# tugitbartlomiej/ViTParticleFilterTracker

Measured on AMD Instinct MI355X. Metric: frames/sec @ 4096 particles, ViT-B/16 224px; 1/2/4/8 MI355X scaling, higher is better.
Workload: dtype bf16; 1 GPU; 4096 particles, vit_base_patch16_224 bf16, 224x224 frames, full tracking step per frame; particles=4096, particles_per_gpu=4096, arch=vit_base_patch16_224, hip_graph=True, parallelism=particle-shard x1

## Files before the change

### vitparticlefiltertracker_amd/csrc/gemm_bf16.hip

```cpp
#include <algorithm>
#include <atomic>
#include "gemm_common.h"

using namespace vpf;
using namespace vpf::gemm;

namespace {

constexpr int BK = 64;
constexpr int OPERAND_BYTES = BM * BK * 2;
static_assert(OPERAND_BYTES == TILE_BYTES, "bf16 K-tile geometry");
constexpr int AUX_PARTS = 15;
constexpr int MAX_PARTS = 16;
constexpr int AUX_BYTES = 2048 + AUX_PARTS * 2048;

template <int EPI, bool WIDE = false, bool OUT8 = false, bool PART = false>
__global__ __launch_bounds__(NTHREADS) void k_gemm_bf16(const bf16_t* __restrict__ A, int lda,
                                                        const bf16_t* __restrict__ W,
                                                        const float* __restrict__ bias,
                                                        const bf16_t* residual,
                                                        const float* __restrict__ pos, int g2,
                                                        const float2* __restrict__ stats,
                                                        const float* __restrict__ colsum,
                                                        bf16_t* C, int ldc, int M, int N, int K, int group,
// ... 120 lines not shown
        }
        return;
    }
    if constexpr (LN) {
        if constexpr (wide) {
            asm volatile("s_waitcnt vmcnt(0)" ::: "memory");
            __builtin_amdgcn_s_barrier();
            asm volatile("" ::: "memory");
        }
        combine_planes(planes_lds, aux, stats_parts, K, ln_eps, tid);
    }
    const int region = (wid >> 1) + ((wid >> 1) >= (nk % 3) ? 1 : 0);
    finish_tile<EPI, OUT8, DIRECT>(smem + region * OPERAND_BYTES + (wid & 1) * 16384, aux, acc, wm, wn, m0, n0, lane,
                                   residual, pos, g2, C, ldc, M, N, stats_out, stats_rows, o8);
}

template <int EPI, bool OUT8 = false>
__global__ __launch_bounds__(NTHREADS) void k_gemm_pp(const bf16_t* __restrict__ A, int lda,
                                                      const bf16_t* __restrict__ W,
                                                      const float* __restrict__ bias,
                                                      const bf16_t* residual,
                                                      const float* __restrict__ pos, int g2,
                                                      const float2* __restrict__ stats,
                                                      const float* __restrict__ colsum,
                                                      bf16_t* C, int ldc, int M, int N, int K, int group,
                                                      int stats_parts, float ln_eps, float* stats_out,
                                                      int stats_rows, Out8 o8) {
    constexpr int HALF = 16384;
    constexpr int RING = 8 * HALF;
    static_assert(RING + AUX_BYTES <= 160 * 1024, "LDS budget");
    __shared__ __attribute__((aligned(16))) char smem[RING + AUX_BYTES];
    const int tid = threadIdx.x, lane = tid & 63;
    const int wid = __builtin_amdgcn_readfirstlane(tid >> 6);
    const int wm = wid >> 2, wn = wid & 3;

    int m0, n0;
    tile_of(M, N, group, m0, n0);
    constexpr bool DIRECT = (EPI == VPF_EPI_LN_GELU || EPI == VPF_EPI_BIAS_GELU) && !OUT8;

    const char* Ablk = reinterpret_cast<const char*>(A) + (size_t)m0 * lda * 2;
    const char* Bblk = reinterpret_cast<const char*>(W) + (size_t)n0 * K * 2;
    uint32_t off[4][2];
#pragma unroll
    for (int p = 0; p < 2; ++p) {
        const int rho = (wid + 8 * p) * 8 + (lane >> 3);
        const int lch = (lane & 7) ^ ((rho >> 1) & 7);
        const int ra0 = (rho >> 6) * 128 + (rho & 63);
        const int rb0 = (rho >> 5) * 64 + (DIRECT ? wperm(rho & 31) : (rho & 31));
        const int ra[2] = {ra0, ra0 + 64}, rb[2] = {rb0, rb0 + 32};
#pragma unroll
        for (int h = 0; h < 2; ++h) {
            off[h == 0 ? 0 : 3][p] = (uint32_t)min(ra[h], M - 1 - m0) * (uint32_t)(lda * 2) + (uint32_t)(lch * 16);
            off[h == 0 ? 1 : 2][p] = (uint32_t)min(rb[h], N - 1 - n0) * (uint32_t)(K * 2) + (uint32_t)(lch * 16);
        }
    }
    const int nk = K / BK;
    auto stage = [&](int type, int kt) {
        kt = min(kt, nk - 1);
        char* slot = smem + ((kt & 1) * 4 + type) * HALF;
        const char* src = (type == 0 || type == 3) ? Ablk : Bblk;
        const uint32_t koff = (uint32_t)kt * (BK * 2);
#pragma unroll
        for (int p = 0; p < 2; ++p)
            __builtin_amdgcn_global_load_lds((gptr_t)(src + off[type][p] + koff), (lptr_t)(slot + (wid + 8 * p) * 1024),
                                             16, 0, 0);
    };

    constexpr bool LN = (EPI == VPF_EPI_LN || EPI == VPF_EPI_LN_GELU);
    char* aux = smem + RING;
    dma_bias_colsum<LN>(aux, bias, colsum, n0, N, wid, lane);
    if constexpr (LN) dma_planes(aux + 2048, stats, stats_parts, m0, M, wid, lane);
    stage(0, 0); stage(1, 0); stage(2, 0); stage(3, 0); stage(0, 1); stage(1, 1);
    asm volatile("s_waitcnt vmcnt(8)" ::: "memory");
    __builtin_amdgcn_s_barrier();
    if (wm == 1) __builtin_amdgcn_s_barrier();
    asm volatile("" ::: "memory");

    f32x4 acc[4][8];
#pragma unroll
    for (int j = 0; j < 4; ++j)
#pragma unroll
        for (int i = 0; i < 8; ++i) acc[j][i] = f32x4{0.f, 0.f, 0.f, 0.f};

    const int fr = lane & 15, fq = lane >> 4;
    const int sw = (fr >> 1) & 7;
    const int abase = (wm * 64 + fr) * 128, bbase = (wn * 32 + fr) * 128;
    auto mfma_quadrant = [&](const i32x4 (&fa)[2][4], const i32x4 (&fb)[2][2], int mh, int nh) {
        asm volatile("s_waitcnt lgkmcnt(0)" ::: "memory");
        __builtin_amdgcn_sched_barrier(0);
#pragma unroll
        for (int ks = 0; ks < 2; ++ks)
#pragma unroll
            for (int j = 0; j < 2; ++j)
#pragma unroll
                for (int i = 0; i < 4; ++i)
                    acc[nh * 2 + j][mh * 4 + i] = __builtin_amdgcn_mfma_f32_16x16x32_bf16(
                        __builtin_bit_cast(bf16x8, fb[ks][j]), __builtin_bit_cast(bf16x8, fa[ks][i]),
                        acc[nh * 2 + j][mh * 4 + i], 0, 0, 0);
        __builtin_amdgcn_sched_barrier(0);
    };
    auto read_a = [&](i32x4 (&fa)[2][4], const char* slot) {
#pragma unroll
        for (int ks = 0; ks < 2; ++ks)
#pragma unroll
            for (int i = 0; i < 4; ++i) fa[ks][i] = lds16(slot + abase + i * 2048 + (((ks * 4 + fq) ^ sw) << 4));
    };
    auto read_b = [&](i32x4 (&fb)[2][2], const char* slot) {
#pragma unroll
        for (int ks = 0; ks < 2; ++ks)
#pragma unroll
            for (int j = 0; j < 2; ++j) fb[ks][j] = lds16(slot + bbase + j * 2048 + (((ks * 4 + fq) ^ sw) << 4));
    };
    auto bar = [&]() {
        __builtin_amdgcn_sched_barrier(0);
        __builtin_amdgcn_s_barrier();
        __builtin_amdgcn_sched_barrier(0);
    };

    for (int kt = 0; kt < nk; ++kt) {
        const char* buf = smem + (kt & 1) * 4 * HALF;
        i32x4 fa0[2][4], fa1[2][4], fb0[2][2], fb1[2][2];
        read_a(fa0, buf);
        read_b(fb0, buf + HALF);
        stage(2, kt + 1);
        asm volatile("s_waitcnt vmcnt(8)" ::: "memory");
        bar();
        mfma_quadrant(fa0, fb0, 0, 0);
        bar();
        read_b(fb1, buf + 2 * HALF);
        stage(3, kt + 1);
        asm volatile("s_waitcnt vmcnt(8)" ::: "memory");
        bar();
        mfma_quadrant(fa0, fb1, 0, 1);
        bar();
        read_a(fa1, buf + 3 * HALF);
        stage(0, kt + 2);
        bar();
        mfma_quadrant(fa1, fb1, 1, 1);
        bar();
        stage(1, kt + 2);
        asm volatile("s_waitcnt vmcnt(8)" ::: "memory");
        bar();
        mfma_quadrant(fa1, fb0, 1, 0);
        bar();
    }
    if (wm == 0) __builtin_amdgcn_s_barrier();
    asm volatile("s_waitcnt vmcnt(0)" ::: "memory");

    if constexpr (LN) combine_planes(aux + 2048, aux, stats_parts, K, ln_eps, tid);
    finish_tile<EPI, OUT8, DIRECT>(smem + wid * 16384, aux, acc, wm, wn, m0, n0, lane, residual, pos, g2, C, ldc, M, N,
                                   stats_out, stats_rows, o8);
}

template <int EPI>
__global__ __launch_bounds__(NTHREADS) void k_gemm_walk(const bf16_t* __restrict__ A, int lda,
                                                        const bf16_t* __restrict__ W,
                                                        const float* __restrict__ bias,
                                                        const float2* __restrict__ stats,
                                                        const float* __restrict__ colsum, bf16_t* C, int ldc, int M,
                                                        int N, int K, int group, int tiles) {
    static_assert(EPI == VPF_EPI_LN_GELU || EPI == VPF_EPI_BIAS_GELU || EPI == VPF_EPI_LN, "FC1's and QKV's epilogues");
    constexpr bool DIRECT = epi_is_gelu(EPI);
    constexpr int HALF = 16384;
    constexpr int RING = 8 * HALF;
    constexpr int AUX_SET = 4096;
    constexpr int GROUP_IMG = 2048;
    __shared__ __attribute__((aligned(16))) char smem[RING + 2 * AUX_SET + (DIRECT ? 0 : 8 * GROUP_IMG)];
    const int tid = threadIdx.x, lane = tid & 63;
    const int wid = __builtin_amdgcn_readfirstlane(tid >> 6);
    const int wm = wid >> 2, wn = wid & 3;
    constexpr bool LN = epi_is_ln(EPI);
    const int nk = K / BK;

    const int stride = (int)gridDim.x >> 3;
    int lid = xcd_first(tiles, (int)blockIdx.x & 7) + ((int)blockIdx.x >> 3);
    const int lid_end = xcd_first(tiles, ((int)blockIdx.x & 7) + 1);
    if (lid >= lid_end) return;
    int m0, n0;
    tile_of_lid(M, N, group, lid, m0, n0);

    const char* Ablk;
    const char* Bblk;
    uint32_t off[4][2];
    auto set_panels = [&](int tm0, int tn0, int ln) {
        Ablk = reinterpret_cast<const char*>(A) + (size_t)tm0 * lda * 2;
        Bblk = reinterpret_cast<const char*>(W) + (size_t)tn0 * K * 2;
#pragma unroll
        for (int p = 0; p < 2; ++p) {
            const int rho = (wid + 8 * p) * 8 + (ln >> 3);
            const int lch = (ln & 7) ^ ((rho >> 1) & 7);
            const int ra0 = (rho >> 6) * 128 + (rho & 63);
            const int rb0 = (rho >> 5) * 64 + (DIRECT ? wperm(rho & 31) : (rho & 31));
            const int ra[2] = {ra0, ra0 + 64}, rb[2] = {rb0, rb0 + 32};
#pragma unroll
            for (int h = 0; h < 2; ++h) {
                off[h == 0 ? 0 : 3][p] = (uint32_t)min(ra[h], M - 1 - tm0) * (uint32_t)(lda * 2) + (uint32_t)(lch * 16);
                off[h == 0 ? 1 : 2][p] = (uint32_t)min(rb[h], N - 1 - tn0) * (uint32_t)(K * 2) + (uint32_t)(lch * 16);
            }
        }
    };
    auto stage = [&](int type, int kt) {
        kt = min(kt, nk - 1);
        char* slot = smem + ((kt & 1) * 4 + type) * HALF;
        const char* src = (type == 0 || type == 3) ? Ablk : Bblk;
        const uint32_t koff = (uint32_t)kt * (BK * 2);
#pragma unroll
        for (int p = 0; p < 2; ++p)
            __builtin_amdgcn_global_load_lds((gptr_t)(src + off[type][p] + koff), (lptr_t)(slot + (wid + 8 * p) * 1024),
                                             16, 0, 0);
    };
    auto load_aux = [&](char* dst, int tm0, int tn0, int ln) {
        dma_bias_colsum<LN>(dst, bias, colsum, tn0, N, wid, ln);
        if constexpr (LN) dma_planes(dst + 2048, stats, 0, tm0, M, wid, ln);
    };

    set_panels(m0, n0, lane);
    load_aux(smem + RING, m0, n0, lane);
    stage(0, 0); stage(1, 0); stage(2, 0); stage(3, 0); stage(0, 1); stage(1, 1);
    asm volatile("s_waitcnt vmcnt(8)" ::: "memory");
    __builtin_amdgcn_s_barrier();
    asm volatile("" ::: "memory");

    f32x4 acc[4][8];
    const int fr = lane & 15, fq = lane >> 4;
    const int sw = (fr >> 1) & 7;
    const int abase = (wm * 64 + fr) * 128, bbase = (wn * 32 + fr) * 128;
    auto mfma_quadrant = [&](const i32x4 (&fa)[2][4], const i32x4 (&fb)[2][2], int mh, int nh) {
        asm volatile("s_waitcnt lgkmcnt(0)" ::: "memory");
        __builtin_amdgcn_sched_barrier(0);
#pragma unroll
        for (int ks = 0; ks < 2; ++ks)
#pragma unroll
            for (int j = 0; j < 2; ++j)
#pragma unroll
                for (int i = 0; i < 4; ++i)
                    acc[nh * 2 + j][mh * 4 + i] = __builtin_amdgcn_mfma_f32_16x16x32_bf16(
                        __builtin_bit_cast(bf16x8, fb[ks][j]), __builtin_bit_cast(bf16x8, fa[ks][i]),
                        acc[nh * 2 + j][mh * 4 + i], 0, 0, 0);
        __builtin_amdgcn_sched_barrier(0);
    };
    auto read_a = [&](i32x4 (&fa)[2][4], const char* slot) {
#pragma unroll
        for (int ks = 0; ks < 2; ++ks)
#pragma unroll
            for (int i = 0; i < 4; ++i) fa[ks][i] = lds16(slot + abase + i * 2048 + (((ks * 4 + fq) ^ sw) << 4));
    };
    auto read_b = [&](i32x4 (&fb)[2][2], const char* slot) {
#pragma unroll
        for (int ks = 0; ks < 2; ++ks)
#pragma unroll
            for (int j = 0; j < 2; ++j) fb[ks][j] = lds16(slot + bbase + j * 2048 + (((ks * 4 + fq) ^ sw) << 4));
    };
    auto bar = [&]() {
        __builtin_amdgcn_sched_barrier(0);
        __builtin_amdgcn_s_barrier();
        __builtin_amdgcn_sched_barrier(0);
    };

    int skt = 0;
    int par = 0;
    for (;;) {
        const int lid_next = lid + stride;
        const bool more = lid_next < lid_end;
        int m0n = m0, n0n = n0;
        if (wm == 1) __builtin_amdgcn_s_barrier();
        asm volatile("" ::: "memory");
#pragma unroll
        for (int j = 0; j < 4; ++j)
#pragma unroll
            for (int i = 0; i < 8; ++i) acc[j][i] = f32x4{0.f, 0.f, 0.f, 0.f};

        for (int kt = 0; kt < nk; ++kt, ++skt) {
            const char* buf = smem + (kt & 1) * 4 * HALF;
            i32x4 fa0[2][4], fa1[2][4], fb0[2][2], fb1[2][2];
            read_a(fa0, buf);
            read_b(fb0, buf + HALF);
            stage(2, skt + 1);
            asm volatile("s_waitcnt vmcnt(8)" ::: "memory");
            bar();
            mfma_quadrant(fa0, fb0, 0, 0);
            bar();
            read_b(fb1, buf + 2 * HALF);
            stage(3, skt + 1);
            asm volatile("s_waitcnt vmcnt(8)" ::: "memory");
            bar();
            mfma_quadrant(fa0, fb1, 0, 1);
            bar();
            if (more && kt == nk - 2) {
                const int ln = opaque_lane();
                tile_of_lid(M, N, group, lid_next, m0n, n0n);
                set_panels(m0n, n0n, ln);
                load_aux(smem + RING + (par ^ 1) * AUX_SET, m0n, n0n, ln);
                skt -= nk;
            }
            read_a(fa1, buf + 3 * HALF);
            stage(0, skt + 2);
            bar();
            mfma_quadrant(fa1, fb1, 1, 1);
            bar();
            stage(1, skt + 2);
            asm volatile("s_waitcnt vmcnt(8)" ::: "memory");
            bar();
            mfma_quadrant(fa1, fb0, 1, 0);
            bar();
        }
        if (wm == 0) __builtin_amdgcn_s_barrier();
        asm volatile("" ::: "memory");
        if constexpr (DIRECT)
            store_wave_tile_direct<EPI, true>(smem + RING + par * AUX_SET, acc, wm, wn, m0, n0, lane, C, ldc, M, N);
        else
            store_wave_tile_group<EPI>(smem + RING + 2 * AUX_SET + wid * GROUP_IMG, smem + RING + par * AUX_SET, acc, wm,
                                       wn, m0, n0, lane, C, ldc, M, N);
        if (!more) break;
        lid = lid_next;
        m0 = m0n;
        n0 = n0n;
        par ^= 1;
    }
    asm volatile("s_waitcnt vmcnt(0)" ::: "memory");
}

}

#define VPF_IS_LN(E) ((E) == VPF_EPI_LN || (E) == VPF_EPI_LN_GELU)
#define VPF_IS_PROD(E) ((E) == VPF_EPI_BIAS_RESIDUAL || (E) == VPF_EPI_PATCH)
#define VPF_GEMM_ARGS                                                                                        \
    A, (int)lda, W, bias, residual, pos, patch_rows, reinterpret_cast<const float2*>(row_stats), colsum, C,     \
        (int)ldc, m, n, k, group, stats_parts, ln_eps, stats_out, stats_rows, o8
#define VPF_GEMM_LAUNCH(E)                                                                                   \
    do {                                                                                                     \
        if (kern == 5 && !(VPF_IS_LN(E) && stats_parts > AUX_PARTS) && o8.q == nullptr)                      \
            hipLaunchKernelGGL((k_gemm_pp<E, false>), grid, block, 0, s, VPF_GEMM_ARGS);                     \
        else if (kern == 5 && VPF_IS_PROD(E) && o8.q != nullptr)                                             \
            hipLaunchKernelGGL((k_gemm_pp<E, VPF_IS_PROD(E)>), grid, block, 0, s, VPF_GEMM_ARGS);            \
        else if (VPF_IS_LN(E) && stats_parts > AUX_PARTS)                                                    \
            hipLaunchKernelGGL((k_gemm_bf16<E, VPF_IS_LN(E)>), grid, block, 0, s, VPF_GEMM_ARGS);             \
        else if (VPF_IS_PROD(E) && o8.q != nullptr)                                                          \
            hipLaunchKernelGGL((k_gemm_bf16<E, false, VPF_IS_PROD(E)>), grid, block, 0, s, VPF_GEMM_ARGS);    \
        else                                                                                                 \
            hipLaunchKernelGGL((k_gemm_bf16<E>), grid, block, 0, s, VPF_GEMM_ARGS);                           \
    } while (0)

constexpr int kDefaultGroup = 4;
static int g_kernel = 0;
static int g_group = -1;
static int gemm_kernel_for(int epilogue) {
    if (g_kernel) return g_kernel;
    return (epilogue == VPF_EPI_LN || epilogue == VPF_EPI_LN_GELU) ? 5 : 1;
}
static int tile_group_for(int64_t N, int epilogue) {
    if (g_group >= 0) return g_group;
    if (N <= 1024) return 2;
    return epilogue == VPF_EPI_LN_GELU ? 8 : kDefaultGroup;
}
int vpf_gemm_tile_group() { return g_group >= 0 ? g_group : kDefaultGroup; }
int vpf_gemm_tile_group_mx8(int epilogue) {
    if (g_group >= 0) return g_group;
    return epilogue == VPF_EPI_LN ? 8 : kDefaultGroup;
}
VPF_API int vpf_gemm_tune(int kernel, int group) {
    if (kernel != 0 && kernel != 1 && kernel != 5) return VPF_ERR_ARG;
    if (group < -1 || group > 64) return VPF_ERR_ARG;
    g_kernel = kernel;
    g_group = kernel == 0 ? -1 : group;
    return 0;
}

static bool walk_by_default(int epilogue) { return epilogue == VPF_EPI_LN_GELU || epilogue == VPF_EPI_LN; }
static int g_walk_mode = 0;
static int g_walk_cap = 0;
static std::atomic<int> g_walk_cus[64];
static int walk_device_grid() {
    int dev = 0;
    if (hipGetDevice(&dev) != hipSuccess || dev < 0 || dev >= 64) return 0;
    int cus = g_walk_cus[dev].load(std::memory_order_relaxed);
    if (cus == 0) {
        if (hipDeviceGetAttribute(&cus, hipDeviceAttributeMultiprocessorCount, dev) != hipSuccess) return 0;
        cus &= ~7;
        g_walk_cus[dev].store(cus, std::memory_order_relaxed);
    }
    return cus;
}
static int walk_grid_for(int epilogue, int64_t tiles, int64_t K, int stats_parts) {
    if (epilogue != VPF_EPI_LN_GELU && epilogue != VPF_EPI_BIAS_GELU && epilogue != VPF_EPI_LN) return 0;
    if (g_kernel != 0 || g_walk_mode < 0 || (g_walk_mode == 0 && !walk_by_default(epilogue))) return 0;
    if ((K / BK) % 2 != 0 || stats_parts != 0 || tiles < 8) return 0;
    int grid = walk_device_grid();
    if (g_walk_cap > 0) grid = std::min(grid, g_walk_cap);
    if (grid < 8) return 0;
    if (g_walk_mode == 0) return tiles >= 2 * (int64_t)grid ? grid : 0;
    return (int)std::min<int64_t>(grid, tiles & ~(int64_t)7);
}
VPF_API int vpf_gemm_persistent(int mode, int grid_cap) {
    if (mode < -1 || mode > 1 || grid_cap < 0 || grid_cap % 8 != 0 || grid_cap > 4096) return VPF_ERR_ARG;
    g_walk_mode = mode;
    g_walk_cap = grid_cap;
    (void)walk_device_grid();
    return 0;
}
VPF_API int vpf_gemm_persistent_grid(int64_t M, int64_t N, int64_t K, int epilogue, int stats_parts) {
    (void)walk_device_grid();
    if (M <= 0 || N <= 0 || K <= 0 || K % BK != 0) return 0;
    const int64_t tiles = ((M + BM - 1) / BM) * ((N + BN - 1) / BN);
    return tiles > INT32_MAX ? 0 : walk_grid_for(epilogue, tiles, K, stats_parts);
}

int vpf_check_out8(const uint8_t* C8, int64_t ld8, const uint32_t* Cs, int64_t lds_c, int64_t rows, int64_t N) {
    if (!C8) return Cs ? VPF_ERR_ARG : 0;
    if (!Cs || N % 128 != 0 || ld8 < N || ld8 % 8 != 0 || ((uintptr_t)C8 & 7) || lds_c < rows || lds_c % 64 != 0 ||
        ((uintptr_t)Cs & 3) || ld8 > INT32_MAX || lds_c > INT32_MAX / 4)
        return VPF_ERR_ARG;
    return 0;
}

int64_t vpf_gemm_check(int64_t M, int64_t N, int64_t K, int64_t k_unit, int64_t lda, int a_align, int a_bytes,
                       bool has_c, int64_t ldc, const float* bias, const float* colsum, const float* row_stats) {
    if (M <= 0 || N <= 0 || K <= 0 || K % k_unit != 0 || N % 8 != 0 || lda < K || lda % a_align != 0) return 0;
    if (has_c && (ldc < N || ldc % 8 != 0 || ldc > INT32_MAX / 2)) return 0;
    if (M > INT32_MAX / 2 || N > 65536 || K > 65536 || lda > INT32_MAX / 2) return 0;
    if ((uint64_t)BM * (uint64_t)lda * (uint64_t)a_bytes > UINT32_MAX) return 0;
    if (((uintptr_t)bias & 15) || ((uintptr_t)colsum & 15) || ((uintptr_t)row_stats & 7)) return 0;
    const int64_t tiles = ((M + BM - 1) / BM) * ((N + BN - 1) / BN);
    return tiles > INT32_MAX ? 0 : tiles;
}

VPF_API int vpf_gemm_bf16(const uint16_t* A, int64_t lda, const uint16_t* W, const float* bias,
                          const uint16_t* residual, const float* pos, int patch_rows, const float* row_stats,
                          const float* colsum, uint16_t* C, int64_t ldc, int64_t M, int64_t N, int64_t K,
                          int epilogue, int stats_parts, float ln_eps, float* stats_out, uint8_t* C8, int64_t ld8,
                          uint32_t* Cs, int64_t lds_c, void* stream) {
    const int64_t tiles = vpf_gemm_check(M, N, K, BK, lda, 8, 2, true, ldc, bias, colsum, row_stats);
    if (!tiles) return VPF_ERR_ARG;
    if (!A || !W || !bias || !C) return VPF_ERR_ARG;
    if (epilogue == VPF_EPI_BIAS_RESIDUAL && !residual) return VPF_ERR_ARG;
    if (epilogue == VPF_EPI_PATCH && (!pos || patch_rows <= 0 || M % patch_rows != 0)) return VPF_ERR_ARG;
    if ((epilogue == VPF_EPI_LN || epilogue == VPF_EPI_LN_GELU) && (!row_stats || !colsum)) return VPF_ERR_ARG;
    if (stats_parts < 0 || stats_parts > MAX_PARTS || !(ln_eps >= 0.f)) return VPF_ERR_ARG;
    if (stats_out && (((uintptr_t)stats_out & 7) || (epilogue != VPF_EPI_BIAS_RESIDUAL && epilogue != VPF_EPI_PATCH)))
        return VPF_ERR_ARG;
    const int64_t srows = epilogue == VPF_EPI_PATCH ? (M / patch_rows) * (patch_rows + 1) : M;
    if (srows > INT32_MAX) return VPF_ERR_ARG;
    const int stats_rows = (int)srows;
    if (C8 && epilogue != VPF_EPI_BIAS_RESIDUAL && epilogue != VPF_EPI_PATCH) return VPF_ERR_ARG;
    if (vpf_check_out8(C8, ld8, Cs, lds_c, srows, N)) return VPF_ERR_ARG;
    const Out8 o8{C8, reinterpret_cast<uint8_t*>(Cs), (int)ld8, (int)lds_c};
    hipStream_t s = (hipStream_t)stream;
    const dim3 grid((unsigned)tiles), block(NTHREADS);
    const int kern = gemm_kernel_for(epilogue);
    const int group = tile_group_for(N, epilogue);
    const int m = (int)M, n = (int)N, k = (int)K;
    if (const int wgrid = C8 ? 0 : walk_grid_for(epilogue, tiles, K, stats_parts)) {
        const float2* st = reinterpret_cast<const float2*>(row_stats);
        if (epilogue == VPF_EPI_LN_GELU)
            hipLaunchKernelGGL((k_gemm_walk<VPF_EPI_LN_GELU>), dim3((unsigned)wgrid), block, 0, s, A, (int)lda, W, bias,
                               st, colsum, C, (int)ldc, m, n, k, group, (int)tiles);
        else if (epilogue == VPF_EPI_LN)
            hipLaunchKernelGGL((k_gemm_walk<VPF_EPI_LN>), dim3((unsigned)wgrid), block, 0, s, A, (int)lda, W, bias, st,
                               colsum, C, (int)ldc, m, n, k, group, (int)tiles);
        else
            hipLaunchKernelGGL((k_gemm_walk<VPF_EPI_BIAS_GELU>), dim3((unsigned)wgrid), block, 0, s, A, (int)lda, W, bias,
                               st, colsum, C, (int)ldc, m, n, k, group, (int)tiles);
        VPF_RETURN_LAUNCH();
    }
    switch (epilogue) {
        case VPF_EPI_BIAS: VPF_GEMM_LAUNCH(VPF_EPI_BIAS); break;
        case VPF_EPI_BIAS_GELU: VPF_GEMM_LAUNCH(VPF_EPI_BIAS_GELU); break;
        case VPF_EPI_BIAS_RESIDUAL: VPF_GEMM_LAUNCH(VPF_EPI_BIAS_RESIDUAL); break;
        case VPF_EPI_PATCH: VPF_GEMM_LAUNCH(VPF_EPI_PATCH); break;
        case VPF_EPI_LN: VPF_GEMM_LAUNCH(VPF_EPI_LN); break;
        case VPF_EPI_LN_GELU: VPF_GEMM_LAUNCH(VPF_EPI_LN_GELU); break;
        default: return VPF_ERR_ARG;
    }
    VPF_RETURN_LAUNCH();
}

template <int EPI>
__global__ __launch_bounds__(256) void k_splitk_reduce(const float* __restrict__ P, int S, int M, int N,
                                                       const float* __restrict__ bias,
                                                       const float2* __restrict__ stats,
                                                       const float* __restrict__ colsum, const bf16_t* residual,
                                                       bf16_t* C, int64_t ldc, float* stats_out) {
    constexpr bool LN = (EPI == VPF_EPI_LN || EPI == VPF_EPI_LN_GELU);
    constexpr bool GELU = (EPI == VPF_EPI_BIAS_GELU || EPI == VPF_EPI_LN_GELU);
    const int per_row = N >> 3;
    const int64_t t = (int64_t)blockIdx.x * blockDim.x + threadIdx.x;
    const bool live = t < (int64_t)M * per_row;
    const int m = live ? (int)(t / per_row) : 0;
    const int n = live ? (int)(t - (int64_t)m * per_row) * 8 : 0;
    float v[8];
    if (live) {
        const float* p = P + (size_t)m * N + n;
        const float4 a0 = *reinterpret_cast<const float4*>(p), a1 = *reinterpret_cast<const float4*>(p + 4);
        v[0] = a0.x; v[1] = a0.y; v[2] = a0.z; v[3] = a0.w; v[4] = a1.x; v[5] = a1.y; v[6] = a1.z; v[7] = a1.w;
        for (int s = 1; s < S; ++s) {
            const float* q = p + (size_t)s * M * N;
            const float4 b0 = *reinterpret_cast<const float4*>(q), b1 = *reinterpret_cast<const float4*>(q + 4);
            v[0] += b0.x; v[1] += b0.y; v[2] += b0.z; v[3] += b0.w; v[4] += b1.x; v[5] += b1.y; v[6] += b1.z; v[7] += b1.w;
        }
        float rstd = 1.f, nrm = 0.f;
        if constexpr (LN) {
            const float2 st = stats[m];
            rstd = st.y;
            nrm = -st.y * st.x;
        }
#pragma unroll
        for (int e = 0; e < 8; ++e) {
            float y = LN ? fmaf(rstd, v[e], fmaf(nrm, colsum[n + e], bias[n + e])) : v[e] + bias[n + e];
            if constexpr (GELU) {
                const f32x2 g = gelu_sig2(f32x2{y, y});
                y = g.x;
            }
            v[e] = y;
        }
    }
    uint32_t o[4];
#pragma unroll
    for (int e = 0; e < 4; ++e) o[e] = pack_bf2(v[2 * e], v[2 * e + 1]);
    if constexpr (EPI == VPF_EPI_BIAS_RESIDUAL) {
        if (live) {
            const uint4 v = add_bf16x8(make_uint4(o[0], o[1], o[2], o[3]),
                                       *reinterpret_cast<const uint4*>(residual + (size_t)m * ldc + n));
            o[0] = v.x; o[1] = v.y; o[2] = v.z; o[3] = v.w;
        }
        if (stats_out != nullptr) {
            float s1 = 0.f, s2 = 0.f;
            if (live) {
#pragma unroll
                for (int e = 0; e < 4; ++e) {
                    const float lo = bf2f((bf16_t)(o[e] & 0xffff)), hi = bf2f((bf16_t)(o[e] >> 16));
                    s1 += lo + hi;
                    s2 = fmaf(lo, lo, s2);
                    s2 = fmaf(hi, hi, s2);
                }
            }
#pragma unroll
            for (int x = 1; x < 8; x <<= 1) {
                s1 += __shfl_xor(s1, x, 64);
                s2 += __shfl_xor(s2, x, 64);
            }
            if (live && (n & 63) == 0)
                *reinterpret_cast<float2*>(stats_out + ((int64_t)(n >> 6) * M + m) * 2) = make_float2(s1, s2);
        }
    }
    if (live) *reinterpret_cast<uint4*>(C + (size_t)m * ldc + n) = make_uint4(o[0], o[1], o[2], o[3]);
}

#define VPF_REDUCE_LAUNCH(E)                                                                                 \
    hipLaunchKernelGGL(k_splitk_reduce<E>, rg, dim3(256), 0, s, partial_ws, splits, m, n, bias, st, colsum, R, Cb, ldc, \
                       stats_out)

VPF_API int vpf_gemm_bf16_splitk(const uint16_t* A, int64_t lda, const uint16_t* W, const float* bias,
                                 const uint16_t* residual, const float* row_stats, const float* colsum, uint16_t* C,
                                 int64_t ldc, int64_t M, int64_t N, int64_t K, int epilogue, int splits,
                                 float* stats_out, float* partial_ws, int64_t ws_elems, void* stream) {
    const bool ln = epilogue == VPF_EPI_LN || epilogue == VPF_EPI_LN_GELU;
    if (splits < 1 || splits > 64) return VPF_ERR_ARG;
    const int64_t tiles = vpf_gemm_check(M, N, K, (int64_t)splits * BK, lda, 8, 2, true, ldc, nullptr, nullptr,
                                         ln ? row_stats : nullptr);
    if (!tiles || tiles > 65535 * 256) return VPF_ERR_ARG;
    if (!A || !W || !bias || !C || !partial_ws || ws_elems < (int64_t)splits * M * N) return VPF_ERR_ARG;
    if (((uintptr_t)partial_ws & 15) || ((uintptr_t)C & 15) || ((uintptr_t)A & 15) || ((uintptr_t)W & 15))
        return VPF_ERR_ARG;
    if (ln && (!row_stats || !colsum)) return VPF_ERR_ARG;
    if (epilogue == VPF_EPI_BIAS_RESIDUAL && (!residual || ((uintptr_t)residual & 15))) return VPF_ERR_ARG;
    if (stats_out && (epilogue != VPF_EPI_BIAS_RESIDUAL || N % 64 != 0 || ((uintptr_t)stats_out & 7)))
        return VPF_ERR_ARG;
    if (epilogue != VPF_EPI_BIAS && epilogue != VPF_EPI_BIAS_GELU && epilogue != VPF_EPI_BIAS_RESIDUAL && !ln)
        return VPF_ERR_ARG;
    hipStream_t s = (hipStream_t)stream;
    const int m = (int)M, n = (int)N, k = (int)K;
    const Out8 o8{nullptr, nullptr, 0, 0};
    hipLaunchKernelGGL((k_gemm_bf16<VPF_EPI_BIAS, false, false, true>),
                       dim3((unsigned)tiles, (unsigned)splits), dim3(NTHREADS), 0, s, reinterpret_cast<const bf16_t*>(A),
                       (int)lda, reinterpret_cast<const bf16_t*>(W), nullptr, nullptr, nullptr, 1, nullptr, nullptr,
                       reinterpret_cast<bf16_t*>(partial_ws), n, m, n, k, vpf_gemm_tile_group(), 0, 0.f, nullptr, m, o8);
    const int e = (int)hipGetLastError();
    if (e) return e;
    const int64_t threads = M * (N / 8);
    const dim3 rg((unsigned)((threads + 255) / 256));
    const float2* st = reinterpret_cast<const float2*>(row_stats);
    const bf16_t* R = reinterpret_cast<const bf16_t*>(residual);
    bf16_t* Cb = reinterpret_cast<bf16_t*>(C);
    switch (epilogue) {
        case VPF_EPI_BIAS: VPF_REDUCE_LAUNCH(VPF_EPI_BIAS); break;
        case VPF_EPI_BIAS_GELU: VPF_REDUCE_LAUNCH(VPF_EPI_BIAS_GELU); break;
        case VPF_EPI_BIAS_RESIDUAL: VPF_REDUCE_LAUNCH(VPF_EPI_BIAS_RESIDUAL); break;
        case VPF_EPI_LN: VPF_REDUCE_LAUNCH(VPF_EPI_LN); break;
        default: VPF_REDUCE_LAUNCH(VPF_EPI_LN_GELU); break;
    }
    VPF_RETURN_LAUNCH();
}
```

### vitparticlefiltertracker_amd/csrc/gemm_common.h

```cpp
#pragma once
#include "vpf_common.h"
#include "mx8.h"
#include "../../include/vpf.h"

int vpf_gemm_tile_group();
int vpf_gemm_tile_group_mx8(int epilogue);
int vpf_check_out8(const uint8_t* C8, int64_t ld8, const uint32_t* Cs, int64_t lds_c, int64_t rows, int64_t N);
int64_t vpf_gemm_check(int64_t M, int64_t N, int64_t K, int64_t k_unit, int64_t lda, int a_align, int a_bytes,
                       bool has_c, int64_t ldc, const float* bias, const float* colsum, const float* row_stats);

namespace vpf {
namespace gemm {

typedef const __attribute__((address_space(1))) void* gptr_t;
typedef __attribute__((address_space(3))) void* lptr_t;
typedef short bf16x8 __attribute__((ext_vector_type(8)));
typedef int i32x4 __attribute__((ext_vector_type(4)));

__device__ __forceinline__ i32x4 lds16(const char* p) {
    i32x4 v;
    asm volatile("ds_read_b128 %0, %1" : "=v"(v) : "v"((uint32_t)(uintptr_t)(lptr_t)p));
    return v;
}
typedef int i32x2 __attribute__((ext_vector_type(2)));
// ... 210 lines not shown
            t.z += u1.x + u1.z; t.w += u1.y + u1.w;
        }
        float* plane = stats_out + (int64_t)(nb >> 6) * stats_rows * 2;
        const int m = mw + 2 * lane;
        if constexpr (PATCH) {
#pragma unroll
            for (int e = 0; e < 2; ++e) {
                const int me = m + e;
                if (me < M) {
                    const int64_t orow = (int64_t)(me / g2) * (g2 + 1) + 1 + me % g2;
                    *reinterpret_cast<float2*>(plane + orow * 2) = e ? make_float2(t.z, t.w) : make_float2(t.x, t.y);
                }
            }
        } else {
            if (m + 1 < M) *reinterpret_cast<float4*>(plane + (int64_t)m * 2) = t;
            else if (m < M) *reinterpret_cast<float2*>(plane + (int64_t)m * 2) = make_float2(t.x, t.y);
        }
    }
}
__device__ __forceinline__ void store_scale_word(Out8 o8, uint32_t word, int mw, int nb, int M, int N, int brick,
                                                 int blk, int r16) {
    const int R = mw + brick * 64;
    if (nb < N && R < M)
        reinterpret_cast<uint32_t*>(o8.s)[(int64_t)(nb >> 7) * o8.lds + R + (((nb >> 5) & 3) + blk) * 16 + r16] = word;
}

template <int EPI>
__device__ __forceinline__ void epi_to_image(char* img, const char* aux, const f32x4 (&acc)[4][8], int wm, int wn,
                                             int lane) {
    constexpr bool LN = epi_is_ln(EPI);
    const int fr = lane & 15, fq = lane >> 4;
    EpiCols cl[4];
    EpiRow rw[8];
#pragma unroll
    for (int j = 0; j < 4; ++j) cl[j] = epi_cols<LN>(aux, wn * 64 + j * 16 + fq * 4);
#pragma unroll
    for (int i = 0; i < 8; ++i) rw[i] = epi_row<LN>(aux, wm * 128 + i * 16 + fr);
#pragma unroll
    for (int j = 0; j < 4; ++j) {
#pragma unroll
        for (int i = 0; i < 8; ++i) epi_to_image4<EPI>(img, i * 16 + fr, j * 4 + fq, acc[j][i], cl[j], rw[i]);
    }
}

template <int EPI>
__device__ __forceinline__ void store_wave_tile_pipe(char* img, const char* aux, const f32x4 (&acc)[4][8], int wm,
                                                     int wn, int m0, int n0, int lane, const uint4 (&res)[16],
                                                     bf16_t* C, int ldc, int M, int N, float* stats_out,
                                                     int stats_rows) {
    constexpr bool LN = epi_is_ln(EPI);
    constexpr bool RES = EPI == VPF_EPI_BIAS_RESIDUAL;
    const int fr = lane & 15, fq = lane >> 4, c16 = lane & 7;
    bf16_t* Cl = C + (int64_t)(m0 + wm * 128 + 2 * (lane >> 3)) * ldc + (n0 + wn * 64 + c16 * 8);
    EpiCols cl[4];
#pragma unroll
    for (int j = 0; j < 4; ++j) cl[j] = epi_cols<LN>(aux, wn * 64 + j * 16 + fq * 4);
#pragma unroll
    for (int i = 0; i < 8; ++i) {
        const EpiRow rw = epi_row<LN>(aux, wm * 128 + i * 16 + fr);
#pragma unroll
        for (int j = 0; j < 4; ++j) epi_to_image4<EPI>(img, i * 16 + fr, j * 4 + fq, acc[j][i], cl[j], rw);
        __builtin_amdgcn_wave_barrier();
#pragma unroll
        for (int h = 0; h < 2; ++h) {
            const int row = i * 16 + 2 * (lane >> 3) + h;
            uint4 v = image_get16(img, row, c16, h == 1);
            const int m = m0 + wm * 128 + row;
            const int n = n0 + wn * 64 + c16 * 8;
            const bool ok = m < M && n < N;
            if constexpr (RES) {
                const uint4 rv = res[2 * i + h];
                const uint32_t w[4] = {v.x, v.y, v.z, v.w};
                const uint32_t rr[4] = {rv.x, rv.y, rv.z, rv.w};
                uint32_t o[4];
#pragma unroll
                for (int e = 0; e < 4; ++e)
                    o[e] = pack_bf2(bf2f((bf16_t)(w[e] & 0xffff)) + bf2f((bf16_t)(rr[e] & 0xffff)),
                                    bf2f((bf16_t)(w[e] >> 16)) + bf2f((bf16_t)(rr[e] >> 16)));
                v = make_uint4(o[0], o[1], o[2], o[3]);
                if (stats_out != nullptr) park_row_partial(img, row, c16, v, ok);
            }
            if (ok) {
                if constexpr (RES) *reinterpret_cast<uint4*>(Cl + (int64_t)(i * 16 + h) * ldc) = v;
                else st16_nt(Cl + (int64_t)(i * 16 + h) * ldc, v);
            }
        }
    }
    if constexpr (RES) {
        const int nb = n0 + wn * 64;
        if (stats_out != nullptr && nb < N) {
            __builtin_amdgcn_wave_barrier();
            float4 t = make_float4(0.f, 0.f, 0.f, 0.f);
#pragma unroll
            for (int q = 0; q < 4; ++q) {
                const float4 u0 = *reinterpret_cast<const float4*>(img + (2 * lane) * 128 + q * 16);
                const float4 u1 = *reinterpret_cast<const float4*>(img + (2 * lane + 1) * 128 + q * 16);
                t.x += u0.x + u0.z; t.y += u0.y + u0.w;
                t.z += u1.x + u1.z; t.w += u1.y + u1.w;
            }
            float* plane = stats_out + (int64_t)(nb >> 6) * stats_rows * 2;
            const int m = m0 + wm * 128 + 2 * lane;
            if (m + 1 < M) *reinterpret_cast<float4*>(plane + (int64_t)m * 2) = t;
            else if (m < M) *reinterpret_cast<float2*>(plane + (int64_t)m * 2) = make_float2(t.x, t.y);
        }
    }
}

__device__ __forceinline__ void lds_write8(const void* p, uint2 v) {
    const i32x2 w = {(int)v.x, (int)v.y};
    asm volatile("ds_write_b64 %0, %1" ::"v"((uint32_t)(uintptr_t)(lptr_t)p), "v"(w) : "memory");
}
template <int EPI>
__device__ __forceinline__ void store_wave_tile_group(char* img, const char* aux, const f32x4 (&acc)[4][8], int wm,
                                                      int wn, int m0, int n0, int lane, bf16_t* C, int ldc, int M,
                                                      int N) {
    static_assert(EPI == VPF_EPI_LN, "group image: the LN fold without GELU (QKV)");
    const int fr = lane & 15, fq = lane >> 4, c16 = lane & 7, r8 = lane >> 3;
    bf16_t* Cl = C + (int64_t)(m0 + wm * 128 + 2 * r8) * ldc + (n0 + wn * 64 + c16 * 8);
    i32x4 cb[4], cc[4];
    i32x2 st[8];
#pragma unroll
    for (int j = 0; j < 4; ++j) {
        const int col = wn * 64 + j * 16 + fq * 4;
        cb[j] = lds16(aux + col * 4);
        cc[j] = lds16(aux + 1024 + col * 4);
    }
#pragma unroll
    for (int i = 0; i < 8; ++i) st[i] = lds8(aux + 2048 + (wm * 128 + i * 16 + fr) * 8);
    asm volatile("s_waitcnt lgkmcnt(0)" : "+v"(cb[0]), "+v"(cb[1]), "+v"(cb[2]), "+v"(cb[3])::"memory");
    asm volatile("" : "+v"(cc[0]), "+v"(cc[1]), "+v"(cc[2]), "+v"(cc[3])::"memory");
    asm volatile("" : "+v"(st[0]), "+v"(st[1]), "+v"(st[2]), "+v"(st[3]), "+v"(st[4]), "+v"(st[5]), "+v"(st[6]),
                   "+v"(st[7])::"memory");
    EpiCols cl[4];
#pragma unroll
    for (int j = 0; j < 4; ++j) cl[j] = EpiCols{__builtin_bit_cast(float4, cb[j]), __builtin_bit_cast(float4, cc[j])};
    const char* wr = img + fr * 128;
    const char* rd = img + (2 * r8) * 128 + ((c16 ^ r8) << 4);
    const int n = n0 + wn * 64 + c16 * 8;
    i32x4 pend[2];
    auto store_group = [&](int i) {
        asm volatile("" : "+v"(pend[0]), "+v"(pend[1])::"memory");
#pragma unroll
        for (int h = 0; h < 2; ++h) {
            uint4 v = __builtin_bit_cast(uint4, pend[h]);
            if (h == 1) { const uint32_t t0 = v.x, t1 = v.y; v.x = v.z; v.y = v.w; v.z = t0; v.w = t1; }
            const int m = m0 + wm * 128 + i * 16 + 2 * r8 + h;
            if (m < M && n < N) st16_nt(Cl + (int64_t)(i * 16 + h) * ldc, v);
        }
    };
#pragma unroll
    for (int i = 0; i < 8; ++i) {
        const float2 s2 = __builtin_bit_cast(float2, st[i]);
        const EpiRow rw = EpiRow{f32x2{s2.y, s2.y}, f32x2{-s2.y * s2.x, -s2.y * s2.x}};
        uint2 pk[4];
#pragma unroll
        for (int j = 0; j < 4; ++j) pk[j] = epi_pack4<EPI>(acc[j][i], cl[j], rw);
#pragma unroll
        for (int j = 0; j < 4; ++j) lds_write8(wr + (((j * 4 + fq) ^ fr) << 3), pk[j]);
        asm volatile("s_waitcnt lgkmcnt(0)" ::: "memory");
        if (i > 0) store_group(i - 1);
        pend[0] = lds16(rd);
        pend[1] = lds16(rd + 128);
    }
    asm volatile("s_waitcnt lgkmcnt(0)" ::: "memory");
    store_group(7);
}

__device__ __forceinline__ int wperm(int r) {
    return (r & ~31) | (((r >> 2) & 3) << 3) | (((r >> 4) & 1) << 2) | (r & 3);
}

template <int EPI, bool DMA_LIVE = false>
__device__ __forceinline__ void store_wave_tile_direct(const char* aux, const f32x4 (&acc)[4][8], int wm, int wn, int m0,
                                                       int n0, int lane, bf16_t* C, int ldc, int M, int N) {
    static_assert(epi_is_gelu(EPI), "direct stores: the GELU epilogues");
    constexpr bool LN = epi_is_ln(EPI);
    const int fr = lane & 15, fq = lane >> 4;
    bf16_t* Cl = C + (int64_t)(m0 + wm * 128 + fr) * ldc + (n0 + wn * 64 + fq * 8);
    EpiCols cl[4];
    EpiRow rws[8];
    if constexpr (DMA_LIVE) {
        i32x4 cb[4], cc[4];
        i32x2 st[8];
#pragma unroll
        for (int j = 0; j < 4; ++j) {
            const int col = wn * 64 + (j >> 1) * 32 + fq * 8 + (j & 1) * 4;
            cb[j] = lds16(aux + col * 4);
            if constexpr (LN) cc[j] = lds16(aux + 1024 + col * 4);
        }
        if constexpr (LN) {
#pragma unroll
            for (int i = 0; i < 8; ++i) st[i] = lds8(aux + 2048 + (wm * 128 + i * 16 + fr) * 8);
        }
        asm volatile("s_waitcnt lgkmcnt(0)" : "+v"(cb[0]), "+v"(cb[1]), "+v"(cb[2]), "+v"(cb[3])::"memory");
        if constexpr (LN) {
            asm volatile("" : "+v"(cc[0]), "+v"(cc[1]), "+v"(cc[2]), "+v"(cc[3])::"memory");
            asm volatile("" : "+v"(st[0]), "+v"(st[1]), "+v"(st[2]), "+v"(st[3]), "+v"(st[4]), "+v"(st[5]), "+v"(st[6]),
                           "+v"(st[7])::"memory");
        }
#pragma unroll
        for (int j = 0; j < 4; ++j) {
            cl[j].b = __builtin_bit_cast(float4, cb[j]);
            cl[j].c = LN ? __builtin_bit_cast(float4, cc[j]) : make_float4(0.f, 0.f, 0.f, 0.f);
        }
#pragma unroll
        for (int i = 0; i < 8; ++i) {
            if constexpr (LN) {
                const float2 s2 = __builtin_bit_cast(float2, st[i]);
                rws[i] = EpiRow{f32x2{s2.y, s2.y}, f32x2{-s2.y * s2.x, -s2.y * s2.x}};
            } else {
                rws[i] = EpiRow{f32x2{1.f, 1.f}, f32x2{0.f, 0.f}};
            }
        }
    } else {
#pragma unroll
        for (int j = 0; j < 4; ++j) cl[j] = epi_cols<LN>(aux, wn * 64 + (j >> 1) * 32 + fq * 8 + (j & 1) * 4);
    }
#pragma unroll
    for (int i = 0; i < 8; ++i) {
        EpiRow rw;
        if constexpr (DMA_LIVE) rw = rws[i];
        else rw = epi_row<LN>(aux, wm * 128 + i * 16 + fr);
        const int m = m0 + wm * 128 + i * 16 + fr;
#pragma unroll
        for (int h = 0; h < 2; ++h) {
            const uint2 lo = epi_pack4<EPI>(acc[2 * h][i], cl[2 * h], rw);
            const uint2 hi = epi_pack4<EPI>(acc[2 * h + 1][i], cl[2 * h + 1], rw);
            const int n = n0 + wn * 64 + h * 32 + fq * 8;
            if (m < M && n < N)
                *reinterpret_cast<uint4*>(Cl + (int64_t)(i * 16) * ldc + h * 32) = make_uint4(lo.x, lo.y, hi.x, hi.y);
        }
    }
}

template <bool PAR = true>
__device__ __forceinline__ void load_residual(uint4 (&res)[16], const bf16_t* residual, int wm, int wn, int m0,
                                              int n0, int lane, int ldc, int M, int N) {
    const int c16 = lane & 7;
    const int n = n0 + wn * 64 + c16 * 8;
    const bf16_t* rl = residual + (int64_t)(m0 + wm * 128 + (PAR ? 2 : 1) * (lane >> 3)) * ldc + n;
#pragma unroll
    for (int it = 0; it < 16; ++it) {
        const int roff = PAR ? (it >> 1) * 16 + (it & 1) : it * 8;
        const int m = m0 + wm * 128 + roff + (PAR ? 2 : 1) * (lane >> 3);
        res[it] = (m < M && n < N) ? *reinterpret_cast<const uint4*>(rl + (int64_t)roff * ldc) : make_uint4(0, 0, 0, 0);
    }
}

template <int EPI, bool OUT8>
__device__ __forceinline__ void store_wave_tile(char* img, const char* aux, const f32x4 (&acc)[4][8], int wm, int wn,
                                                int m0, int n0, int lane, const uint4 (&res)[16],
                                                const float* __restrict__ pos, int g2, bf16_t* C, int ldc, int M,
                                                int N, float* stats_out, int stats_rows, Out8 o8) {
    epi_to_image<EPI>(img, aux, acc, wm, wn, lane);
    const int c16 = lane & 7;
    constexpr bool PROD = (EPI == VPF_EPI_BIAS_RESIDUAL || EPI == VPF_EPI_PATCH);
    constexpr bool GATHER8 = OUT8 && EPI != VPF_EPI_PATCH;
    uint32_t e8s[16];
    __builtin_amdgcn_wave_barrier();
#pragma unroll
    for (int it = 0; it < 16; ++it) {
        const int row = it * 8 + (lane >> 3);
        uint4 v = image_get16(img, row, c16, row & 1);
        const int m = m0 + wm * 128 + row;
        const int n = n0 + wn * 64 + c16 * 8;
        const bool ok = m < M && n < N;
        int64_t orow = m;
        if constexpr (EPI == VPF_EPI_PATCH) {
            const int pi = m % g2;
            orow = (int64_t)(m / g2) * (g2 + 1) + 1 + pi;
            const float* pr = pos + (int64_t)(1 + pi) * N + min(n, N - 8);
            const float4 p0 = *reinterpret_cast<const float4*>(pr);
            const float4 p1 = *reinterpret_cast<const float4*>(pr + 4);
            const uint32_t w[4] = {v.x, v.y, v.z, v.w};
            const float pv[8] = {p0.x, p0.y, p0.z, p0.w, p1.x, p1.y, p1.z, p1.w};
            uint32_t o[4];
#pragma unroll
            for (int e = 0; e < 4; ++e)
                o[e] = pack_bf2(bf2f((bf16_t)(w[e] & 0xffff)) + pv[2 * e], bf2f((bf16_t)(w[e] >> 16)) + pv[2 * e + 1]);
            v = make_uint4(o[0], o[1], o[2], o[3]);
        }
        if constexpr (EPI == VPF_EPI_BIAS_RESIDUAL) v = add_bf16x8(v, res[it]);
        if constexpr (PROD) {
            if (stats_out != nullptr) park_row_partial(img, row, c16, v, ok);
        }
        if constexpr (OUT8) {
            uint32_t e8;
            const uint2 q = mx8_quant8(v, e8);
            e8s[it] = e8;
            if (ok) {
                *reinterpret_cast<uint2*>(o8.q + orow * o8.ldq + n) = q;
                if (!GATHER8 && (c16 & 3) == 0) o8.s[mx8_scale_byte(orow, n, o8.lds)] = (uint8_t)e8;
            }
        }
        if (ok && C != nullptr) *reinterpret_cast<uint4*>(C + orow * ldc + n) = v;
    }
    if constexpr (GATHER8) {
        __builtin_amdgcn_wave_barrier();
        if ((c16 & 3) == 0) {
#pragma unroll
            for (int it = 0; it < 16; ++it) {
                const int row = it * 8 + (lane >> 3);
                const int w = (row >> 6) * 32 + (c16 >> 2) * 16 + (row & 15);
                img[(w >> 4) * 128 + 64 + (w & 15) * 4 + ((row >> 4) & 3)] = (char)e8s[it];
            }
        }
// ... 110 lines not shown
```

Before: 7.676 frames/s.

## Route bias+residual GEMMs through persistent walk kernel with fused row-stat planes

Extends the persistent tile-walking GEMM kernel to the bias+residual epilogue used by the attention-projection and FC2 GEMMs (K/64 of 12 or 48). It adds a residual-aware grouped store that adds the residual in bf16 and emits per-row sum and sum-of-squares partials for the next LayerNorm via DPP reductions. The aim is to overlap the next tile's prologue with the epilogue and to avoid a separate stats pass. The cost is extra register pressure for 16 prefetched residual vectors and new stats-plane write logic.

```diff
diff --git a/vitparticlefiltertracker_amd/csrc/gemm_bf16.hip b/vitparticlefiltertracker_amd/csrc/gemm_bf16.hip
--- a/vitparticlefiltertracker_amd/csrc/gemm_bf16.hip
+++ b/vitparticlefiltertracker_amd/csrc/gemm_bf16.hip
@@ -296,20 +296,26 @@
                                    stats_out, stats_rows, o8);
 }
 
+constexpr int WALK_HALF = 16384;
+constexpr int WALK_RING = 8 * WALK_HALF;
+constexpr int WALK_GROUP_IMG = 2048;
+constexpr int walk_aux_set(int epi) { return epi == VPF_EPI_BIAS_RESIDUAL ? 1024 : 4096; }
+constexpr int walk_smem(int epi) {
+    return WALK_RING + 2 * walk_aux_set(epi) + (epi_is_gelu(epi) ? 0 : 8 * WALK_GROUP_IMG);
+}
+
 template <int EPI>
-__global__ __launch_bounds__(NTHREADS) void k_gemm_walk(const bf16_t* __restrict__ A, int lda,
-                                                        const bf16_t* __restrict__ W,
-                                                        const float* __restrict__ bias,
-                                                        const float2* __restrict__ stats,
-                                                        const float* __restrict__ colsum, bf16_t* C, int ldc, int M,
-                                                        int N, int K, int group, int tiles) {
-    static_assert(EPI == VPF_EPI_LN_GELU || EPI == VPF_EPI_BIAS_GELU || EPI == VPF_EPI_LN, "FC1's and QKV's epilogues");
+__device__ __forceinline__ void gemm_walk_body(char* smem, const bf16_t* __restrict__ A, int lda,
+                                               const bf16_t* __restrict__ W, const float* __restrict__ bias,
+                                               const float2* __restrict__ stats, const float* __restrict__ colsum,
+                                               const bf16_t* residual, bf16_t* C, int ldc, int M, int N, int K,
+                                               int group, int tiles, float* stats_out) {
+    constexpr bool RES = EPI == VPF_EPI_BIAS_RESIDUAL;
     constexpr bool DIRECT = epi_is_gelu(EPI);
-    constexpr int HALF = 16384;
-    constexpr int RING = 8 * HALF;
-    constexpr int AUX_SET = 4096;
-    constexpr int GROUP_IMG = 2048;
-    __shared__ __attribute__((aligned(16))) char smem[RING + 2 * AUX_SET + (DIRECT ? 0 : 8 * GROUP_IMG)];
+    constexpr int HALF = WALK_HALF;
+    constexpr int RING = WALK_RING;
+    constexpr int AUX_SET = walk_aux_set(EPI);
+    constexpr int GROUP_IMG = WALK_GROUP_IMG;
     const int tid = threadIdx.x, lane = tid & 63;
     const int wid = __builtin_amdgcn_readfirstlane(tid >> 6);
     const int wm = wid >> 2, wn = wid & 3;
@@ -448,10 +454,19 @@
             mfma_quadrant(fa1, fb0, 1, 0);
             bar();
         }
+        [[maybe_unused]] uint4 res[16];
+        [[maybe_unused]] int eln = lane;
+        if constexpr (RES) {
+            eln = opaque_lane();
+            load_residual<true>(res, residual, wm, wn, m0, n0, eln, ldc, M, N);
+        }
         if (wm == 0) __builtin_amdgcn_s_barrier();
         asm volatile("" ::: "memory");
         if constexpr (DIRECT)
             store_wave_tile_direct<EPI, true>(smem + RING + par * AUX_SET, acc, wm, wn, m0, n0, lane, C, ldc, M, N);
+        else if constexpr (RES)
+            store_wave_tile_group_res(smem + RING + 2 * AUX_SET + wid * GROUP_IMG, smem + RING + par * AUX_SET, acc, wm,
+                                      wn, m0, n0, eln, res, C, ldc, M, N, stats_out, M);
         else
             store_wave_tile_group<EPI>(smem + RING + 2 * AUX_SET + wid * GROUP_IMG, smem + RING + par * AUX_SET, acc, wm,
                                        wn, m0, n0, lane, C, ldc, M, N);
@@ -462,6 +477,28 @@
         par ^= 1;
     }
     asm volatile("s_waitcnt vmcnt(0)" ::: "memory");
+}
+
+template <int EPI>
+__global__ __launch_bounds__(NTHREADS) void k_gemm_walk(const bf16_t* __restrict__ A, int lda,
+                                                        const bf16_t* __restrict__ W,
+                                                        const float* __restrict__ bias,
+                                                        const float2* __restrict__ stats,
+                                                        const float* __restrict__ colsum, bf16_t* C, int ldc, int M,
+                                                        int N, int K, int group, int tiles) {
+    static_assert(EPI == VPF_EPI_LN_GELU || EPI == VPF_EPI_BIAS_GELU || EPI == VPF_EPI_LN, "FC1's and QKV's epilogues");
+    __shared__ __attribute__((aligned(16))) char smem[walk_smem(EPI)];
+    gemm_walk_body<EPI>(smem, A, lda, W, bias, stats, colsum, nullptr, C, ldc, M, N, K, group, tiles, nullptr);
+}
+
+__global__ __launch_bounds__(NTHREADS) void k_gemm_walk_res(const bf16_t* __restrict__ A, int lda,
+                                                            const bf16_t* __restrict__ W,
+                                                            const float* __restrict__ bias, const bf16_t* residual,
+                                                            bf16_t* C, int ldc, int M, int N, int K, int group,
+                                                            int tiles, float* stats_out) {
+    __shared__ __attribute__((aligned(16))) char smem[walk_smem(VPF_EPI_BIAS_RESIDUAL)];
+    gemm_walk_body<VPF_EPI_BIAS_RESIDUAL>(smem, A, lda, W, bias, nullptr, nullptr, residual, C, ldc, M, N, K, group,
+                                          tiles, stats_out);
 }
 
 }
@@ -510,7 +547,10 @@
     return 0;
 }
 
-static bool walk_by_default(int epilogue) { return epilogue == VPF_EPI_LN_GELU || epilogue == VPF_EPI_LN; }
+static bool walk_by_default(int epilogue, int64_t nk) {
+    if (epilogue == VPF_EPI_BIAS_RESIDUAL) return nk == 12 || nk == 48;
+    return epilogue == VPF_EPI_LN_GELU || epilogue == VPF_EPI_LN;
+}
 static int g_walk_mode = 0;
 static int g_walk_cap = 0;
 static std::atomic<int> g_walk_cus[64];
@@ -526,8 +566,10 @@
     return cus;
 }
 static int walk_grid_for(int epilogue, int64_t tiles, int64_t K, int stats_parts) {
-    if (epilogue != VPF_EPI_LN_GELU && epilogue != VPF_EPI_BIAS_GELU && epilogue != VPF_EPI_LN) return 0;
-    if (g_kernel != 0 || g_walk_mode < 0 || (g_walk_mode == 0 && !walk_by_default(epilogue))) return 0;
+    if (epilogue != VPF_EPI_LN_GELU && epilogue != VPF_EPI_BIAS_GELU && epilogue != VPF_EPI_LN &&
+        epilogue != VPF_EPI_BIAS_RESIDUAL)
+        return 0;
+    if (g_kernel != 0 || g_walk_mode < 0 || (g_walk_mode == 0 && !walk_by_default(epilogue, K / BK))) return 0;
     if ((K / BK) % 2 != 0 || stats_parts != 0 || tiles < 8) return 0;
     int grid = walk_device_grid();
     if (g_walk_cap > 0) grid = std::min(grid, g_walk_cap);
@@ -595,7 +637,10 @@
     const int m = (int)M, n = (int)N, k = (int)K;
     if (const int wgrid = C8 ? 0 : walk_grid_for(epilogue, tiles, K, stats_parts)) {
         const float2* st = reinterpret_cast<const float2*>(row_stats);
-        if (epilogue == VPF_EPI_LN_GELU)
+        if (epilogue == VPF_EPI_BIAS_RESIDUAL)
+            hipLaunchKernelGGL(k_gemm_walk_res, dim3((unsigned)wgrid), block, 0, s, A, (int)lda, W, bias, residual, C,
+                               (int)ldc, m, n, k, group, (int)tiles, stats_out);
+        else if (epilogue == VPF_EPI_LN_GELU)
             hipLaunchKernelGGL((k_gemm_walk<VPF_EPI_LN_GELU>), dim3((unsigned)wgrid), block, 0, s, A, (int)lda, W, bias,
                                st, colsum, C, (int)ldc, m, n, k, group, (int)tiles);
         else if (epilogue == VPF_EPI_LN)
diff --git a/vitparticlefiltertracker_amd/csrc/gemm_common.h b/vitparticlefiltertracker_amd/csrc/gemm_common.h
--- a/vitparticlefiltertracker_amd/csrc/gemm_common.h
+++ b/vitparticlefiltertracker_amd/csrc/gemm_common.h
@@ -386,6 +386,91 @@
     for (int i = 0; i < 8; ++i) {
         const float2 s2 = __builtin_bit_cast(float2, st[i]);
         const EpiRow rw = EpiRow{f32x2{s2.y, s2.y}, f32x2{-s2.y * s2.x, -s2.y * s2.x}};
+        uint2 pk[4];
+#pragma unroll
+        for (int j = 0; j < 4; ++j) pk[j] = epi_pack4<EPI>(acc[j][i], cl[j], rw);
+#pragma unroll
+        for (int j = 0; j < 4; ++j) lds_write8(wr + (((j * 4 + fq) ^ fr) << 3), pk[j]);
+        asm volatile("s_waitcnt lgkmcnt(0)" ::: "memory");
+        if (i > 0) store_group(i - 1);
+        pend[0] = lds16(rd);
+        pend[1] = lds16(rd + 128);
+    }
+    asm volatile("s_waitcnt lgkmcnt(0)" ::: "memory");
+    store_group(7);
+}
+
+__device__ __forceinline__ float2 row_partial8(uint4 v, bool ok) {
+    typedef __bf16 bf16x2_t __attribute__((ext_vector_type(2)));
+    const uint32_t w[4] = {v.x, v.y, v.z, v.w};
+    const bf16x2_t one2 = __builtin_bit_cast(bf16x2_t, 0x3F803F80u);
+    float s1 = 0.f, s2 = 0.f;
+#pragma unroll
+    for (int e = 0; e < 4; ++e) {
+        const bf16x2_t pr = __builtin_bit_cast(bf16x2_t, w[e]);
+        s1 = __builtin_amdgcn_fdot2_f32_bf16(pr, one2, s1, false);
+        s2 = __builtin_amdgcn_fdot2_f32_bf16(pr, pr, s2, false);
+    }
+    if (!ok) { s1 = 0.f; s2 = 0.f; }
+    return make_float2(s1, s2);
+}
+template <int SHL>
+__device__ __forceinline__ float dpp_row_shl(float x) {
+    return __builtin_bit_cast(float, __builtin_amdgcn_update_dpp(0, __builtin_bit_cast(int, x), 0x100 + SHL, 0xF, 0xF, true));
+}
+__device__ __forceinline__ float row8_sum(float p) {
+    const float q = p + dpp_row_shl<1>(p);
+    float t = 0.f;
+    t += q;
+    t += dpp_row_shl<2>(q);
+    t += dpp_row_shl<4>(q);
+    t += dpp_row_shl<6>(q);
+    return t;
+}
+__device__ __forceinline__ void store_wave_tile_group_res(char* img, const char* aux, const f32x4 (&acc)[4][8], int wm,
+                                                          int wn, int m0, int n0, int lane, const uint4 (&res)[16],
+                                                          bf16_t* C, int ldc, int M, int N, float* stats_out,
+                                                          int stats_rows) {
+    constexpr int EPI = VPF_EPI_BIAS_RESIDUAL;
+    const int fr = lane & 15, fq = lane >> 4, c16 = lane & 7, r8 = lane >> 3;
+    bf16_t* Cl = C + (int64_t)(m0 + wm * 128 + 2 * r8) * ldc + (n0 + wn * 64 + c16 * 8);
+    i32x4 cb[4];
+#pragma unroll
+    for (int j = 0; j < 4; ++j) cb[j] = lds16(aux + (wn * 64 + j * 16 + fq * 4) * 4);
+    asm volatile("s_waitcnt lgkmcnt(0)" : "+v"(cb[0]), "+v"(cb[1]), "+v"(cb[2]), "+v"(cb[3])::"memory");
+    EpiCols cl[4];
+#pragma unroll
+    for (int j = 0; j < 4; ++j) cl[j] = EpiCols{__builtin_bit_cast(float4, cb[j]), make_float4(0.f, 0.f, 0.f, 0.f)};
+    const EpiRow rw = EpiRow{f32x2{1.f, 1.f}, f32x2{0.f, 0.f}};
+    const char* wr = img + fr * 128;
+    const char* rd = img + (2 * r8) * 128 + ((c16 ^ r8) << 4);
+    const int n = n0 + wn * 64 + c16 * 8;
+    const int nb = n0 + wn * 64;
+    const bool planes = stats_out != nullptr && nb < N;
+    float* pl = stats_out + ((int64_t)(nb >> 6) * stats_rows + (m0 + wm * 128 + 2 * r8)) * 2;
+    i32x4 pend[2];
+    auto store_group = [&](int i) {
+        asm volatile("" : "+v"(pend[0]), "+v"(pend[1])::"memory");
+        const int m = m0 + wm * 128 + i * 16 + 2 * r8;
+        uint4 v[2];
+#pragma unroll
+        for (int h = 0; h < 2; ++h) {
+            v[h] = __builtin_bit_cast(uint4, pend[h]);
+            if (h == 1) { const uint32_t t0 = v[h].x, t1 = v[h].y; v[h].x = v[h].z; v[h].y = v[h].w; v[h].z = t0; v[h].w = t1; }
+            v[h] = add_bf16x8(v[h], res[2 * i + h]);
+            if (m + h < M && n < N) *reinterpret_cast<uint4*>(Cl + (int64_t)(i * 16 + h) * ldc) = v[h];
+        }
+        if (planes) {
+            const float2 p0 = row_partial8(v[0], m < M && n < N), p1 = row_partial8(v[1], m + 1 < M && n < N);
+            const float4 t = make_float4(row8_sum(p0.x), row8_sum(p0.y), row8_sum(p1.x), row8_sum(p1.y));
+            if (c16 == 0) {
+                if (m + 1 < M) *reinterpret_cast<float4*>(pl + i * 32) = t;
+                else if (m < M) *reinterpret_cast<float2*>(pl + i * 32) = make_float2(t.x, t.y);
+            }
+        }
+    };
+#pragma unroll
+    for (int i = 0; i < 8; ++i) {
         uint2 pk[4];
 #pragma unroll
         for (int j = 0; j < 4; ++j) pk[j] = epi_pack4<EPI>(acc[j][i], cl[j], rw);
```

Result: faster. 7.829 frames/s, median of 6 (+2.0%).
